# vbronetskyi/nclt-slam-project

Measured on AMD Instinct MI355X. Metric: relocalization frames/sec @640x480, 10k-landmark DB; Hamming-match HBM GB/s, higher is better.
Workload: dtype u8; 1 GPU; 640x480 BGR frames, 10000-record landmark DB (640000 descriptors, rows=fixed64), global relocalization tick per frame: ORB(500) + whole-DB mutual Hamming scan + top-25 PnP-RANSAC(200); frames resident in HBM, every frame's 96-byte result record written to pinned host memory by the tick's last kernel; distinct_frames=32, preroll_steps=20, streams=4, records=10000, descriptors=640000, parallelism=frames sharded across ranks, database replicated, no collective

## Files before the change

### nclt-slam-project_amd/csrc/reloc_ctx.hip

```cpp
#include <stdarg.h>
#include <stdlib.h>

#include "reloc_internal.h"

static thread_local char g_err[512] = "";

void reloc_set_error(const char *fmt, ...)
{
    va_list ap;
    va_start(ap, fmt);
    vsnprintf(g_err, sizeof(g_err), fmt, ap);
    va_end(ap);
}

RELOC_API const char *reloc_last_error(void) { return g_err; }

RELOC_API int reloc_device_count(void)
{
    int n = 0;
    if (hipGetDeviceCount(&n) != hipSuccess) return 0;
    return n;
}

template <typename T>
// ... 14 lines not shown
        pyr += ((w + 63) / 64 * 64) * h + 256;
    }
    c->pyr_bytes = pyr;
    rc |= dalloc(&c->pyr, pyr);
    rc |= dalloc(&c->blur, pyr);
    rc |= dalloc(&c->nms, pyr);
    rc |= dalloc(&c->rz_tab, (int64_t)NLEV * 2 * 2 * (c->max_w > c->max_h ? c->max_w : c->max_h));
    rc |= dalloc((char **)&c->pyr_tiles, (int64_t)((c->max_w + 15) / 16) * ((c->max_h + 15) / 16) * 128);
    rc |= dalloc(&c->hist, NLEV * 256);
    rc |= dalloc(&c->cand_cnt, NLEV);
    rc |= dalloc(&c->cand_key, (int64_t)NLEV * RELOC_ORB_STAGE1_CAP);
    rc |= dalloc(&c->cand_resp, (int64_t)NLEV * RELOC_ORB_STAGE1_CAP);
    rc |= dalloc(&c->kp_cnt, NLEV);
    rc |= dalloc(&c->kp_key, (int64_t)NLEV * RELOC_ORB_STAGE1_CAP);
    rc |= dalloc(&c->kp_resp, (int64_t)NLEV * RELOC_ORB_STAGE1_CAP);
    rc |= dalloc(&c->f_xy, mf * 2);
    rc |= dalloc(&c->f_size, mf);
    rc |= dalloc(&c->f_angle, mf);
    rc |= dalloc(&c->f_resp, mf);
    rc |= dalloc(&c->f_oct, mf);
    rc |= dalloc(&c->f_desc, mf * 32);
    rc |= dalloc(&c->f_count, 1);
    rc |= dalloc(&c->frame_img, (int64_t)c->max_w * c->max_h * 3);
    rc |= dalloc((char **)&c->orb_const, 1024);
    rc |= dalloc(&c->dbg_cut, NLEV);
    rc |= dalloc(&c->cand_ids, MAX_CAND);
    rc |= dalloc(&c->cand_n, 1);
    rc |= dalloc(&c->m_qidx, (int64_t)MAX_CAND * MAX_REC_ROWS);
    rc |= dalloc(&c->m_tidx, (int64_t)MAX_CAND * MAX_REC_ROWS);
    rc |= dalloc(&c->m_dist, (int64_t)MAX_CAND * MAX_REC_ROWS);
    rc |= dalloc(&c->m_n, MAX_CAND);
    rc |= dalloc(&c->p_obj, (int64_t)MAX_CAND * MAX_REC_ROWS * 3);
    rc |= dalloc(&c->p_img, (int64_t)MAX_CAND * MAX_REC_ROWS * 2);
    rc |= dalloc(&c->p_Rt, (int64_t)MAX_CAND * MAX_HYP * 12);
    rc |= dalloc(&c->p_cnt, (int64_t)MAX_CAND * MAX_HYP);
    rc |= dalloc(&c->p_inl, (int64_t)MAX_CAND * MAX_REC_ROWS);
    rc |= dalloc(&c->p_out, MAX_CAND);
    rc |= dalloc(&c->tick_res, 1);
    if (hipHostMalloc((void **)&c->tick_res_host, sizeof(TickResult), hipHostMallocDefault) != hipSuccess) {
        reloc_set_error("hipHostMalloc(result record) failed");
        c->tick_res_host = nullptr;
        rc |= RELOC_E_HIP;
    } else memset(c->tick_res_host, 0, sizeof(TickResult));
    rc |= dalloc(&c->accum_res, 1);
    rc |= dalloc(&c->tick_flags, 4);
    rc |= dalloc(&c->scan_ticket, (8 * 8 + 1) * 32);
    if (rc == 0 && hipMemset(c->scan_ticket, 0, (8 * 8 + 1) * 32 * 4) != hipSuccess) rc = RELOC_E_HIP;
    return rc;
}

int g_reloc_live_contexts = 0;

RELOC_API reloc_ctx *reloc_create(int device, int max_w, int max_h, int max_feat)
{
    int n = 0;
    if (hipGetDeviceCount(&n) != hipSuccess || n <= 0) {
        reloc_set_error("no HIP device available (libreloc_hip has no CPU fallback)");
        return nullptr;
    }
    if (device < 0 || device >= n || max_w < 64 || max_h < 64 || max_feat < 64) {
        reloc_set_error("reloc_create: bad arguments (device %d of %d, %dx%d, max_feat %d)", device, n,
                        max_w, max_h, max_feat);
        return nullptr;
    }
    if (hipSetDevice(device) != hipSuccess) {
        reloc_set_error("hipSetDevice(%d) failed", device);
        return nullptr;
    }
    reloc_ctx *c = new reloc_ctx();
    __atomic_add_fetch(&g_reloc_live_contexts, 1, __ATOMIC_RELAXED);
    c->device = device;
    c->max_w = max_w;
    c->max_h = max_h;
    c->max_feat = max_feat;
    hipDeviceProp_t prop;
    if (hipGetDeviceProperties(&prop, device) == hipSuccess) c->num_cu = prop.multiProcessorCount;
    if (hipStreamCreateWithFlags(&c->own_stream, hipStreamNonBlocking) != hipSuccess ||
        hipEventCreate(&c->t0) != hipSuccess || hipEventCreate(&c->t1) != hipSuccess) {
        reloc_set_error("stream/event creation failed");
        __atomic_sub_fetch(&g_reloc_live_contexts, 1, __ATOMIC_RELAXED);
        delete c;
        return nullptr;
    }
    c->stream = c->own_stream;
    c->prm.nfeatures = 500;
    c->prm.max_candidates = RELOC_MAX_CANDIDATES;
    c->prm.min_matches = RELOC_MIN_MATCHES;
    c->prm.min_inliers = RELOC_MIN_INLIERS;
    c->prm.ransac_iterations = RELOC_RANSAC_ITERATIONS;
    c->prm.global_max_candidates = RELOC_GLOBAL_MAX_CANDIDATES;
    c->prm.global_min_inliers = RELOC_GLOBAL_MIN_INLIERS;
    c->prm.accum_min_kpts = RELOC_ACCUM_MIN_KPTS;
    c->prm.candidate_radius_m = RELOC_CANDIDATE_RADIUS_M;
// ... 12 lines not shown
        if (const char *e = getenv("RELOC_SCAN_GENS")) c->scan_gens = atoi(e);
        if (const char *e = getenv("RELOC_LOCAL_TWO_STAGE")) c->local_two_stage = atoi(e) != 0;
    }
    if (ctx_alloc(c) != 0) {
        reloc_destroy(c);
        return nullptr;
    }
    return c;
}

RELOC_API void reloc_destroy(reloc_ctx *c)
{
    if (!c) return;
    (void)hipSetDevice(c->device);
    if (c->stream) (void)hipStreamSynchronize(c->stream);
    db_arrays_drop(c->db_share, c->db_desc, c->db_pts3d, c->db_kp2d, c->db_off, c->db_pose, c->db_xy_heading);
    void *ptrs[] = {c->pyr, c->blur, c->nms, c->rz_tab, c->pyr_tiles, c->hist, c->cand_cnt, c->cand_key, c->cand_resp,
                    c->kp_cnt, c->kp_key, c->kp_resp, c->f_xy, c->f_size, c->f_angle, c->f_resp, c->f_oct,
                    c->f_desc, c->f_count, c->frame_img, c->orb_const, c->dbg_cut, c->db_counts, c->topk_part, c->cand_ids, c->cand_n, c->m_qidx,
                    c->m_tidx, c->m_dist, c->m_n, c->p_obj, c->p_img, c->p_Rt, c->p_cnt, c->p_inl,
                    c->p_out, c->tick_res, c->accum_res, c->tick_flags, c->scan_ticket, c->clahe_plane, c->clahe_lut,
                    c->rect_xy };
    for (void *p : ptrs)
        if (p) (void)hipFree(p);
    if (c->tick_res_host) (void)hipHostFree(c->tick_res_host);
    {
        DbArena &a = c->db_slot[1 - c->db_sel];
        db_arrays_drop(a.share, a.desc, a.pts3d, a.kp2d, a.off, a.pose, a.xy_heading);
        if (a.counts) (void)hipFree(a.counts);
        if (a.topk_part) (void)hipFree(a.topk_part);
    }
    for (int i = 0; i < 8; ++i)
        if (c->scratch[i]) (void)hipFree(c->scratch[i]);
    for (int k = 0; k < RELOC_PROF_N; ++k)
        if (c->prof[k].init)
            for (int i = 0; i < RELOC_PROF_RING; ++i) {
                (void)hipEventDestroy(c->prof[k].a[i]);
                (void)hipEventDestroy(c->prof[k].b[i]);
            }
    if (c->t0) (void)hipEventDestroy(c->t0);
    if (c->t1) (void)hipEventDestroy(c->t1);
    if (c->own_stream) (void)hipStreamDestroy(c->own_stream);
    __atomic_sub_fetch(&g_reloc_live_contexts, 1, __ATOMIC_RELAXED);
    delete c;
}

RELOC_API int reloc_get_params(reloc_ctx *c, reloc_params *out)
{
    ARG_CHECK_CTX(c, out, "reloc_get_params");
    *out = c->prm;
    return RELOC_OK;
}

RELOC_API int reloc_set_params(reloc_ctx *c, const reloc_params *p)
{
    ARG_CHECK_CTX(c, p, "reloc_set_params");
// ... 2 lines not shown
    ARG_CHECK(p->global_max_candidates >= 1 && p->global_max_candidates <= MAX_CAND, "global_max_candidates must be in [1, 32]");
    ARG_CHECK(p->ransac_iterations >= 1 && p->ransac_iterations <= MAX_HYP, "ransac_iterations must be in [1, 1024]");
    ARG_CHECK(p->min_matches >= RELOC_PNP_SAMPLE && p->min_inliers >= 0 && p->global_min_inliers >= 0 && p->accum_min_kpts >= 1,
              "min_matches must be >= 4, inlier / keypoint gates non-negative");
    ARG_CHECK(p->candidate_radius_m >= 0 && p->heading_tol_deg >= 0 && p->heading_tol_deg <= 180 && p->ransac_reproj_px > 0 &&
                  p->ransac_confidence > 0 && p->ransac_confidence < 1 && p->consistency_m >= 0 && p->accum_min_dist_m >= 0,
              "a gate is out of range");
    ARG_CHECK((p->gray_coeff_bits == RELOC_GRAY_SHIFT || p->gray_coeff_bits == RELOC_GRAY15_SHIFT) && p->reserved0 == 0,
              "gray_coeff_bits must be 14 or 15, reserved0 must be 0");
    c->prm = *p;
    return RELOC_OK;
}

RELOC_API int reloc_set_stream(reloc_ctx *c, void *hip_stream)
{
    ARG_CHECK_CTX(c, true, "ctx is NULL");
    c->stream = hip_stream ? (hipStream_t)hip_stream : c->own_stream;
    return RELOC_OK;
}

RELOC_API int reloc_sync(reloc_ctx *c)
{
    ARG_CHECK_CTX(c, true, "ctx is NULL");
    HIP_TRY(hipStreamSynchronize(c->stream));
    return RELOC_OK;
}

RELOC_API void *reloc_dev_alloc(reloc_ctx *c, int64_t bytes)
{
    if (!c || bytes < 0) { reloc_set_error("reloc_dev_alloc: bad arguments"); return nullptr; }
    void *p = nullptr;
    (void)hipSetDevice(c->device);
    if (hipMalloc(&p, (size_t)(bytes > 0 ? bytes : 1)) != hipSuccess) {
        reloc_set_error("hipMalloc(%lld) failed", (long long)bytes);
        return nullptr;
    }
    return p;
}

RELOC_API int reloc_dev_free(reloc_ctx *c, void *p)
{
    ARG_CHECK_CTX(c, true, "ctx is NULL");
    if (p) HIP_TRY(hipFree(p));
    return RELOC_OK;
}

RELOC_API int reloc_h2d(reloc_ctx *c, void *dst, const void *src, int64_t bytes)
{
    ARG_CHECK_CTX(c, dst && src && bytes >= 0, "reloc_h2d");
    HIP_TRY(hipMemcpyAsync(dst, src, (size_t)bytes, hipMemcpyHostToDevice, c->stream));
    return RELOC_OK;
}

RELOC_API int reloc_d2d(reloc_ctx *c, void *dst, const void *src, int64_t bytes)
{
    ARG_CHECK_CTX(c, dst && src && bytes >= 0, "reloc_d2d");
    HIP_TRY(hipMemcpyAsync(dst, src, (size_t)bytes, hipMemcpyDeviceToDevice, c->stream));
    return RELOC_OK;
}

RELOC_API int reloc_set_exclusive(reloc_ctx *c, int on)
{
    ARG_CHECK_CTX(c, true, "ctx is NULL");
    c->exclusive_hint = on < 0 ? -1 : (on != 0);
// ... 8 lines not shown
        return nullptr;
    }
    return p;
}

RELOC_API int reloc_host_free(void *p)
{
    if (p) HIP_TRY(hipHostFree(p));
    return RELOC_OK;
}

RELOC_API void *reloc_get_stream(reloc_ctx *c) { return c ? (void *)c->stream : nullptr; }

RELOC_API int reloc_d2h(reloc_ctx *c, void *dst, const void *src, int64_t bytes)
{
    ARG_CHECK_CTX(c, dst && src && bytes >= 0, "reloc_d2h");
    HIP_TRY(hipMemcpyAsync(dst, src, (size_t)bytes, hipMemcpyDeviceToHost, c->stream));
    return RELOC_OK;
}

RELOC_API int reloc_timer_begin(reloc_ctx *c)
{
    ARG_CHECK_CTX(c, true, "ctx is NULL");
    HIP_TRY(hipEventRecord(c->t0, c->stream));
    return RELOC_OK;
}

RELOC_API int reloc_timer_end(reloc_ctx *c, float *ms)
{
    ARG_CHECK_CTX(c, ms, "reloc_timer_end");
    HIP_TRY(hipEventRecord(c->t1, c->stream));
// ... 76 lines not shown
```

### nclt-slam-project_amd/csrc/reloc_internal.h

```cpp
#pragma once
#include <hip/hip_runtime.h>
#include <stdint.h>
#include <stdio.h>
#include <string.h>

#include "../../include/reloc.h"
#include "../../include/reloc_spec.h"

#define RELOC_API extern "C" __attribute__((visibility("default")))
#define RELOC_PROF_RING 256

void reloc_set_error(const char *fmt, ...);

#define HIP_TRY(expr)                                                                      \
    do {                                                                                   \
        hipError_t e_ = (expr);                                                            \
        if (e_ != hipSuccess) {                                                            \
            reloc_set_error("%s failed: %s (%s:%d)", #expr, hipGetErrorString(e_), __FILE__, \
                            __LINE__);                                                     \
            return RELOC_E_HIP;                                                            \
        }                                                                                  \
    } while (0)

#define ARG_CHECK(cond, msg)                                 \
    do {                                                     \
        if (!(cond)) {                                       \
            reloc_set_error("bad argument: %s", msg);        \
            return RELOC_E_ARG;                              \
        }                                                    \
    } while (0)

#define ARG_CHECK_CTX(c, cond, msg)                           \
    do {                                                      \
        if (!(c) || !(cond)) {                                \
            reloc_set_error("bad argument: %s", msg);         \
            return RELOC_E_ARG;                               \
        }                                                     \
        (void)hipSetDevice((c)->device);                      \
    } while (0)

constexpr int NLEV = RELOC_ORB_NLEVELS;
constexpr int MAX_REC_ROWS = 4096;
constexpr int MAX_CAND = 32;
constexpr int MAX_HYP = 1024;
constexpr int64_t MAX_DB_RECORDS = 0xFFFFF;

#ifndef RELOC_SCAN_NUM_VGPR
#define RELOC_SCAN_NUM_VGPR 104
#endif
#if RELOC_SCAN_NUM_VGPR > 0
#define RELOC_SCAN_VGPR_ATTR __attribute__((amdgpu_num_vgpr(RELOC_SCAN_NUM_VGPR / 2)))
#else
#define RELOC_SCAN_VGPR_ATTR
#endif
#ifndef RELOC_SMALL_PRIO
#define RELOC_SMALL_PRIO 3
#endif
#define RELOC_SMALL_KERNEL_PRIO() __builtin_amdgcn_s_setprio(RELOC_SMALL_PRIO)

struct OrbLevel {
    int w, h;
    int stride;
    int64_t off;
    float scale;
    int quota;
};

struct TickResult {
// ... 235 lines not shown
    int32_t *cand_ids = nullptr;
    int32_t *cand_n = nullptr;
    int32_t *m_qidx = nullptr, *m_tidx = nullptr, *m_dist = nullptr, *m_n = nullptr;
    float *p_obj = nullptr, *p_img = nullptr;
    double *p_Rt = nullptr;
    int32_t *p_cnt = nullptr;
    int32_t *p_inl = nullptr;
    PnpOut *p_out = nullptr;
    int exclusive_hint = -1;
    bool local_two_stage = false;
    TickResult *tick_res = nullptr;
    TickResult *tick_res_host = nullptr;
    bool tick_failed = false;
    int32_t tick_seq = 0;
    TickResult *tick_res_ext = nullptr;
};

int reloc_scratch(reloc_ctx *ctx, int slot, int64_t bytes, void **out);
void reloc_prof_begin(reloc_ctx *ctx, int which);
void reloc_prof_end(reloc_ctx *ctx, int which);

void db_arrays_drop(DbShare *&share, uint8_t *&desc, float *&pts3d, float *&kp2d, int64_t *&off, double *&pose, double *&xyh);
extern int g_reloc_live_contexts;
static inline bool ctx_alone(const reloc_ctx *c)
{
    return c->exclusive_hint > 0 || (c->exclusive_hint < 0 && __atomic_load_n(&g_reloc_live_contexts, __ATOMIC_RELAXED) == 1);
}

constexpr int RELOC_BATCH_MAX = 8;

template <typename Fn>
// ... 18 lines not shown
```

### nclt-slam-project_amd/csrc/reloc_match.hip

```cpp
#include <stdlib.h>
#include <new>
#include <type_traits>
#include <utility>

#include "reloc_internal.h"

typedef uint32_t u32;

__device__ __forceinline__ u32 bcnt_acc(u32 x, u32 acc)
{
    u32 r;
    asm("v_bcnt_u32_b32 %0, %1, %2" : "=v"(r) : "v"(x), "v"(acc));
    return r;
}
__device__ __forceinline__ u32 min_u16(u32 a, u32 b)
{
    u32 r;
    asm("v_min_u16 %0, %1, %2" : "=v"(r) : "v"(a), "v"(b));
    return r;
}
template <u32 IDX>
__device__ __forceinline__ u32 key_fma(u32 d, u32 c128)
{
    u32 r;
// ... 448 lines not shown
        if (atomicAdd(&ticket_pool[words * TICKET_STRIDE], 1u) == gridDim.x - 1) {
            for (int x = 0; x <= words; ++x)
                __hip_atomic_store(&ticket_pool[x * TICKET_STRIDE], 0u, __ATOMIC_RELAXED, __HIP_MEMORY_SCOPE_AGENT);
        }
    }
}

template <int NJ, bool EMIT, int NW>
__global__ __launch_bounds__(64 * NW, 16 / NW) RELOC_SCAN_VGPR_ATTR void k_db_scan(
    const uint4 *__restrict__ db, const int64_t *__restrict__ off, const int32_t *__restrict__ rec_ids,
    const int32_t *__restrict__ n_ids_p, int n_ids_max, const uint4 *__restrict__ cur,
    const int32_t *__restrict__ n_cur_p, int n_cur_max, int max_rows, int32_t *__restrict__ counts,
    int32_t *__restrict__ m_qidx, int32_t *__restrict__ m_tidx, int32_t *__restrict__ m_dist,
    int32_t *__restrict__ m_n, int emit_stride, ScanMask mask, u32 *ticket, int quota, int n_bounded, int col_words)
{
    extern __shared__ u32 lds[];
    if constexpr (EMIT) RELOC_SMALL_KERNEL_PRIO();
    const int C = n_cur_p ? min(*n_cur_p, n_cur_max) : n_cur_max;
    if constexpr (EMIT)
        db_scan_body<NJ, true, NW>(lds, C, db, off, rec_ids, n_ids_p, n_ids_max, cur, max_rows, counts, m_qidx, m_tidx, m_dist, m_n,
                                   emit_stride, mask, ticket, quota);
    else
        db_count_body<NJ, NW>(lds, C, db, off, rec_ids, n_ids_p, n_ids_max, cur, max_rows, counts, mask, ticket, quota, n_bounded, col_words);
}

struct EmitFrame {
    const int32_t *rec_ids, *n_ids_p; const uint4 *cur; const int32_t *n_cur_p;
    int32_t *m_qidx, *m_tidx, *m_dist, *m_n; const float *g_xy; float *g_obj, *g_img;
};
struct EmitBatch { EmitFrame f[RELOC_BATCH_MAX]; };
static EmitFrame emit_frame(const reloc_ctx *c)
{
    EmitFrame F;
    F.rec_ids = c->cand_ids; F.n_ids_p = c->cand_n; F.cur = (const uint4 *)c->f_desc; F.n_cur_p = c->f_count;
    F.m_qidx = c->m_qidx; F.m_tidx = c->m_tidx; F.m_dist = c->m_dist; F.m_n = c->m_n; F.g_xy = c->f_xy; F.g_obj = c->p_obj; F.g_img = c->p_img;
    return F;
}

__global__ __launch_bounds__(256, 4) RELOC_SCAN_VGPR_ATTR void k_db_emit_batch(const uint4 *__restrict__ db, const int64_t *__restrict__ off, int n_ids_max,
                                                          int n_cur_max, int max_rows, int emit_stride, const float *__restrict__ g_pts3d,
                                                          EmitBatch bt)
{
    extern __shared__ u32 lds[];
    RELOC_SMALL_KERNEL_PRIO();
    const EmitFrame &F = bt.f[blockIdx.y];
    ScanMask mask;
    mask.g_pts3d = g_pts3d; mask.g_xy = F.g_xy; mask.g_obj = F.g_obj; mask.g_img = F.g_img;
    const int C = F.n_cur_p ? min(*F.n_cur_p, n_cur_max) : n_cur_max;
    db_scan_body<8, true, 4>(lds, C, db, off, F.rec_ids, F.n_ids_p, n_ids_max, F.cur, max_rows, nullptr, F.m_qidx, F.m_tidx, F.m_dist, F.m_n,
                             emit_stride, mask, nullptr, 0);
}

static int scan_lds_bytes(const char *who, int col_words, int max_rows, size_t &lds)
{
// ... 397 lines not shown
    if (n_ids_max <= 0) return RELOC_OK;
    if (n_cur_max > 65535) { reloc_set_error("db scan: more than 65535 current descriptors"); return RELOC_E_CAPACITY; }
    if (max_rows > MAX_REC_ROWS) { reloc_set_error("db scan: record larger than %d rows", MAX_REC_ROWS); return RELOC_E_CAPACITY; }
    if (max_rows < 1) max_rows = 1;
    const int nj = n > 1 || n_cur_max > 256 ? 8 : (n_cur_max <= 128 ? 2 : 4);
    const int cb = 64 * nj;
    const int ncb = (n_cur_max + cb - 1) / cb > 0 ? (n_cur_max + cb - 1) / cb : 1;
    size_t lds;
    if (int rc = scan_lds_bytes("db scan", ncb * cb, max_rows, lds)) return rc;
    const int grid = n_ids_max < c0->num_cu * 16 ? n_ids_max : c0->num_cu * 16;
    if (n == 1) {
        const EmitFrame &F = bt.f[0];
        ScanMask mask;
        mask.g_pts3d = g_pts3d; mask.g_xy = F.g_xy; mask.g_obj = F.g_obj; mask.g_img = F.g_img;
#define RELOC_LAUNCH_EMIT(NJ, NW)                                                                                            \
    hipLaunchKernelGGL((k_db_scan<NJ, true, NW>), dim3(grid), dim3(64 * NW), lds, c0->stream, (const uint4 *)db_desc, db_off, F.rec_ids, \
                       F.n_ids_p, n_ids_max, F.cur, F.n_cur_p, n_cur_max, max_rows, nullptr, F.m_qidx, F.m_tidx, F.m_dist, F.m_n,  \
                       emit_stride, mask, nullptr, 0, 0, ncb * cb)
        if (latency) {
            if (nj == 2) RELOC_LAUNCH_EMIT(2, 8); else if (nj == 4) RELOC_LAUNCH_EMIT(4, 8); else RELOC_LAUNCH_EMIT(8, 8);
        } else {
            if (nj == 2) RELOC_LAUNCH_EMIT(2, 4); else if (nj == 4) RELOC_LAUNCH_EMIT(4, 4); else RELOC_LAUNCH_EMIT(8, 4);
        }
#undef RELOC_LAUNCH_EMIT
    } else {
        hipLaunchKernelGGL(k_db_emit_batch, dim3(grid, n), dim3(256), lds, c0->stream, (const uint4 *)db_desc, db_off, n_ids_max,
                           n_cur_max, max_rows, emit_stride, g_pts3d, bt);
    }
    HIP_TRY(hipGetLastError());
    return RELOC_OK;
}

int launch_tick_emit(reloc_ctx *const *ctxs, int n, bool latency)
// ... 531 lines not shown
static void db_store_slot(reloc_ctx *ctx)
{
    DbArena &a = ctx->db_slot[ctx->db_sel];
    a.cap_records = ctx->db_cap_records; a.cap_rows = ctx->db_cap_rows; a.records = ctx->db_records; a.rows = ctx->db_rows;
    a.max_rows = ctx->db_max_rows; a.desc = ctx->db_desc; a.pts3d = ctx->db_pts3d; a.kp2d = ctx->db_kp2d; a.off = ctx->db_off;
    a.pose = ctx->db_pose; a.xy_heading = ctx->db_xy_heading; a.counts = ctx->db_counts; a.topk_part = ctx->topk_part;
    a.topk_blocks = ctx->topk_blocks;
    a.share = ctx->db_share;
}

RELOC_API int reloc_db_share(reloc_ctx *dst, reloc_ctx *src)
{
    ARG_CHECK_CTX(dst, src && src != dst, "reloc_db_share");
    if (src->device != dst->device) { reloc_set_error("reloc_db_share: contexts live on different devices"); return RELOC_E_ARG; }
    if (!db_ready(src)) { reloc_set_error("reloc_db_share: the source context has no database"); return RELOC_E_STATE; }
    HIP_TRY(hipStreamSynchronize(dst->stream));
    HIP_TRY(hipStreamSynchronize(src->stream));
    int32_t *counts = nullptr;
    unsigned long long *topk = nullptr;
    const int blocks = (int)((src->db_cap_records + 1023) / 1024);
    if (hipMalloc((void **)&counts, (size_t)src->db_cap_records * 4) != hipSuccess ||
        hipMalloc((void **)&topk, (size_t)blocks * 32 * sizeof(unsigned long long)) != hipSuccess) {
        if (counts) (void)hipFree(counts);
        reloc_set_error("reloc_db_share: scratch allocation failed");
        return RELOC_E_HIP;
    }
    if (dst->db_shared) db_unshare(dst);
    else {
        if (dst->db_counts) (void)hipFree(dst->db_counts);
        if (dst->topk_part) (void)hipFree(dst->topk_part);
// ... 100 lines not shown
```

### nclt-slam-project_amd/csrc/reloc_tick.hip

```cpp
#include <time.h>

#include "reloc_internal.h"

struct TickParams {
    double base_pose[7];
    double b2c_t[3];
    double b2c_R[9];
    int mode;
    int check_consistency;
    int n_records;
    int max_candidates, min_matches, min_inliers, global_min_inliers;
    double radius_m, cos_tol, reproj_max_px, global_reproj_max_px, consistency_m;
    int seq;
};

__device__ void rot_to_quat(const double R[9], double q[4])
{
    const double tr = R[0] + R[4] + R[8];
    double qx, qy, qz, qw;
    if (tr > 0) {
        const double s = 0.5 / sqrt(tr + 1.0);
        qw = 0.25 / s;
        qx = (R[7] - R[5]) * s; qy = (R[2] - R[6]) * s; qz = (R[3] - R[1]) * s;
    } else if (R[0] > R[4] && R[0] > R[8]) {
// ... 477 lines not shown
    p.check_consistency = check_consistency;
    p.n_records = (int)ctx->db_records;
    const reloc_params &q = ctx->prm;
    p.max_candidates = q.max_candidates; p.min_matches = q.min_matches; p.min_inliers = q.min_inliers;
    p.global_min_inliers = q.global_min_inliers;
    p.radius_m = q.candidate_radius_m; p.cos_tol = heading_cos_tol_host(ctx); p.reproj_max_px = q.reproj_max_px;
    p.global_reproj_max_px = q.global_reproj_max_px; p.consistency_m = q.consistency_m;
    p.seq = 0;
    return p;
}

static int tick_next_seq(reloc_ctx *ctx)
{
    ctx->tick_seq = ctx->tick_seq >= 0x7fffffff ? 1 : ctx->tick_seq + 1;
    ctx->tick_failed = false;
    return ctx->tick_seq;
}

struct SetCandBatch { int32_t *cand_ids[RELOC_BATCH_MAX], *cand_n[RELOC_BATCH_MAX], *flags[RELOC_BATCH_MAX]; };
__global__ void k_set_candidates_batch(const int32_t *__restrict__ ids, int k, SetCandBatch b, int flag)
{
    const int f = blockIdx.x;
    if (threadIdx.x == 0) {
        int m = 0;
        for (int i = 0; i < k; ++i)
            if (ids[f * k + i] >= 0) b.cand_ids[f][m++] = ids[f * k + i];
        *b.cand_n[f] = m;
        *b.flags[f] = flag;
    }
}
// ... 152 lines not shown
    int rc;
    if (cand_dev) {
        SetCandBatch sb;
        frame_slots(ctxs, n, [&](int f, reloc_ctx *c, int) { sb.cand_ids[f] = c->cand_ids; sb.cand_n[f] = c->cand_n; sb.flags[f] = c->tick_flags; });
        hipLaunchKernelGGL(k_set_candidates_batch, dim3(n), dim3(64), 0, c0->stream, cand_dev, k, sb, mode == RELOC_TICK_LOCAL ? 0 : 1);
    }
    if ((rc = launch_tick_emit(ctxs, n, latency))) return rc;
    if ((rc = pnp_run_candidates(ctxs, n, seeds, latency))) return rc;
    FinalBatch b;
    frame_slots(ctxs, n, [&](int f, reloc_ctx *c, int g) {
        b.f[f] = final_frame(c, base_poses + 7 * g, res_ext_base ? res_ext_base + g : c->tick_res_ext, f < n ? tick_next_seq(c) : 0);
    });
    return launch_tick_finalize(ctxs, n, b, make_tick_params(c0, base_poses, mode, check_consistency));
}

static int tick_run(reloc_ctx *const *ctxs, int n, const uint8_t *const *imgs, int w, int h, int order, const double *base_poses,
                    int mode, const uint64_t *seeds)
{
    reloc_ctx *c0 = ctxs[0];
    if (c0->max_feat > 65535) { reloc_set_error("tick: max_feat must be <= 65535"); return RELOC_E_CAPACITY; }
    const bool latency = tick_latency(ctxs, n, mode);
    int rc;
    if ((rc = orb_run(ctxs, n, imgs, w, h, w * 3, 3, order, c0->prm.nfeatures, latency))) return rc;
    if (mode != RELOC_TICK_GLOBAL)
        for (int f = 0; f < n; ++f) launch_candidates_local(ctxs[f], make_tick_params(ctxs[f], base_poses + 7 * f, mode, -1));
    if (mode != RELOC_TICK_LOCAL) {
        if ((rc = scan_counts(ctxs, n, base_poses, mode == RELOC_TICK_AUTO))) return rc;
        TopkBatch b;
        frame_slots(ctxs, n, [&](int f, reloc_ctx *c, int) { b.f[f] = topk_frame(c, c->cand_ids, nullptr, nullptr, mode == RELOC_TICK_AUTO); });
        launch_topk_counts(ctxs, n, b, c0->prm.global_max_candidates, 0);
    }
    return solve_run(ctxs, n, nullptr, 0, base_poses, mode, -1, seeds, nullptr);
}

static int scan_run(reloc_ctx *const *ctxs, int n, const uint8_t *const *imgs, int w, int h, int order, const double *base_poses,
                    const TopkBatch &out, int k, int id_base)
{
    int rc;
    if ((rc = orb_run(ctxs, n, imgs, w, h, w * 3, 3, order, ctxs[0]->prm.nfeatures, tick_latency(ctxs, n, RELOC_TICK_GLOBAL))))
        return rc;
    if ((rc = scan_counts(ctxs, n, base_poses, false))) return rc;
    launch_topk_counts(ctxs, n, out, k, id_base);
    HIP_TRY(hipGetLastError());
    return RELOC_OK;
}

RELOC_API int reloc_tick_dev(reloc_ctx *ctx, const uint8_t *img_dev, int w, int h, int order, const double base_pose[7],
                             int global_reloc, uint64_t seed)
{
    tick_mark_failed(&ctx, 1);
    ARG_CHECK_CTX(ctx, img_dev && base_pose && w >= 64 && h >= 64 && global_reloc >= 0 && global_reloc <= 2, "reloc_tick_dev");
    if (int rc = ctx_batch_check(&ctx, 1, "reloc_tick_dev")) return rc;
    return tick_run(&ctx, 1, &img_dev, w, h, order, base_pose, global_reloc, &seed);
}

RELOC_API int reloc_tick_batch_dev(reloc_ctx *const *ctxs, int n, const uint8_t *const *imgs_dev, int w, int h, int order,
                                   const double *base_poses, int global_reloc, const uint64_t *seeds)
{
    tick_mark_failed(ctxs, n);
    ARG_CHECK(ctxs && imgs_dev && base_poses && n >= 1 && n <= 8 && w >= 64 && h >= 64 && global_reloc >= 0 && global_reloc <= 2,
              "reloc_tick_batch_dev");
    for (int f = 0; f < n; ++f) ARG_CHECK(imgs_dev[f], "reloc_tick_batch_dev: NULL frame");
    if (int rc = ctx_batch_check(ctxs, n, "reloc_tick_batch_dev")) return rc;
    return tick_run(ctxs, n, imgs_dev, w, h, order, base_poses, global_reloc, seeds);
}

RELOC_API int reloc_tick_wait(reloc_ctx *ctx)
{
    ARG_CHECK_CTX(ctx, true, "ctx is NULL");
    if (ctx->tick_failed) {
        reloc_set_error("reloc_tick_wait: the last tick on this context failed before its result record was enqueued");
        return RELOC_E_STATE;
    }
    const int want = ctx->tick_seq;
    if (want == 0 || !ctx->tick_res_host) { HIP_TRY(hipStreamSynchronize(ctx->stream)); return RELOC_OK; }
    volatile int32_t *stamp = (volatile int32_t *)&ctx->tick_res_host->pad[0];
    struct timespec t0;
    clock_gettime(CLOCK_MONOTONIC, &t0);
    for (unsigned spin = 1;; ++spin) {
        if (*stamp == want) { __atomic_thread_fence(__ATOMIC_ACQUIRE); return RELOC_OK; }
        __builtin_ia32_pause();
        if ((spin & 0x3FF) == 0) {
            struct timespec t1;
            clock_gettime(CLOCK_MONOTONIC, &t1);
            if ((t1.tv_sec - t0.tv_sec) * 1000000000ll + (t1.tv_nsec - t0.tv_nsec) > 20000000ll) break;
        }
    }
    HIP_TRY(hipStreamSynchronize(ctx->stream));
    if (*stamp != want) { reloc_set_error("reloc_tick_wait: the stream drained without the tick's result record (a tick that failed to enqueue?)"); return RELOC_E_STATE; }
    return RELOC_OK;
}

RELOC_API int reloc_tick_result(reloc_ctx *ctx, double anchor_pose[7], int32_t *n_inl, float *reproj, int32_t *lm_idx,
                                int32_t *outcome, int32_t *n_candidates)
{
    ARG_CHECK_CTX(ctx, true, "ctx is NULL");
    { const int rc = reloc_tick_wait(ctx); if (rc) return rc; }
    const TickResult r = *ctx->tick_res_host;
    if (anchor_pose) for (int k = 0; k < 7; ++k) anchor_pose[k] = r.anchor_pose[k];
    if (n_inl) *n_inl = r.n_inl;
    if (reproj) *reproj = (float)r.reproj;
    if (lm_idx) *lm_idx = r.lm_idx;
    if (outcome) *outcome = r.outcome;
    if (n_candidates) *n_candidates = r.n_candidates;
    return RELOC_OK;
}

RELOC_API const void *reloc_tick_result_dev(reloc_ctx *ctx) { return ctx ? ctx->tick_res : nullptr; }

RELOC_API int reloc_tick_result_to(reloc_ctx *ctx, void *pinned_record)
{
    ARG_CHECK_CTX(ctx, true, "ctx is NULL");
    ctx->tick_res_ext = (TickResult *)pinned_record;
    return RELOC_OK;
}

RELOC_API int reloc_tick_result_ex(reloc_ctx *ctx, double anchor_pose[7], int32_t *n_inl, double *reproj, int32_t *lm_idx,
                                   int32_t *outcome, int32_t *n_candidates, int32_t *n_features, int32_t *relocating)
{
    ARG_CHECK_CTX(ctx, true, "ctx is NULL");
    { const int rc = reloc_tick_wait(ctx); if (rc) return rc; }
    const TickResult r = *ctx->tick_res_host;
    if (anchor_pose) for (int k = 0; k < 7; ++k) anchor_pose[k] = r.anchor_pose[k];
    if (n_inl) *n_inl = r.n_inl;
    if (reproj) *reproj = r.reproj;
    if (lm_idx) *lm_idx = r.lm_idx;
    if (outcome) *outcome = r.outcome;
    if (n_candidates) *n_candidates = r.n_candidates;
    if (n_features) *n_features = r.n_features;
    if (relocating) *relocating = r.relocating;
    return RELOC_OK;
}

RELOC_API int reloc_tick(reloc_ctx *ctx, const uint8_t *img, int w, int h, int order, const double base_pose[7],
                         int global_reloc, uint64_t seed, double anchor_pose[7], int32_t *n_inl, float *reproj,
                         int32_t *lm_idx, int32_t *outcome, int32_t *n_candidates)
{
    ARG_CHECK_CTX(ctx, img && base_pose && w >= 64 && h >= 64, "reloc_tick");
    if (w > ctx->max_w || h > ctx->max_h) { reloc_set_error("frame exceeds ctx capacity"); return RELOC_E_CAPACITY; }
    HIP_TRY(hipMemcpyAsync(ctx->frame_img, img, (size_t)w * h * 3, hipMemcpyHostToDevice, ctx->stream));
    int rc = reloc_tick_dev(ctx, ctx->frame_img, w, h, order, base_pose, global_reloc, seed);
    if (rc) return rc;
    return reloc_tick_result(ctx, anchor_pose, n_inl, reproj, lm_idx, outcome, n_candidates);
}

RELOC_API int reloc_tick_scan_dev(reloc_ctx *ctx, const uint8_t *img_dev, int w, int h, int order, const double base_pose[7],
                                  int32_t *topk_ids_dev, int32_t *topk_counts_dev, int k)
{
    ARG_CHECK_CTX(ctx, img_dev && topk_ids_dev && topk_counts_dev && k > 0 && k <= MAX_CAND && w >= 64 && h >= 64,
              "reloc_tick_scan_dev");
    if (int rc = ctx_batch_check(&ctx, 1, "reloc_tick_scan_dev")) return rc;
    TopkBatch out;
    frame_slots(&ctx, 1, [&](int f, reloc_ctx *c, int) { out.f[f] = topk_frame(c, topk_ids_dev, topk_counts_dev, nullptr, false); });
// ... 3 lines not shown
RELOC_API int reloc_tick_solve_dev(reloc_ctx *ctx, const int32_t *cand_ids_dev, int n_cand, const double base_pose[7],
                                   int check_consistency, uint64_t seed)
{
    tick_mark_failed(&ctx, 1);
    ARG_CHECK_CTX(ctx, cand_ids_dev && base_pose && n_cand >= 0 && n_cand <= MAX_CAND, "reloc_tick_solve_dev");
    if (int rc = ctx_batch_check(&ctx, 1, "reloc_tick_solve_dev")) return rc;
    return solve_run(&ctx, 1, cand_ids_dev, n_cand, base_pose, check_consistency ? RELOC_TICK_LOCAL : RELOC_TICK_GLOBAL,
                     check_consistency, &seed, nullptr);
}

RELOC_API int reloc_shard_scan_batch_dev(reloc_ctx *const *ctxs, int n, const uint8_t *const *imgs_dev, int w, int h, int order,
                                         const double *base_poses, int k, int64_t id_base, int32_t *scan_out_dev)
{
    int rc = ctx_batch_check(ctxs, n, "reloc_shard_scan_batch_dev");
    if (rc) return rc;
    ARG_CHECK(imgs_dev && scan_out_dev && k > 0 && k <= MAX_CAND && w >= 64 && h >= 64 && id_base >= 0 &&
              id_base + ctxs[0]->db_records <= 0x7fffffff, "reloc_shard_scan_batch_dev");
    for (int f = 0; f < n; ++f) ARG_CHECK(imgs_dev[f], "reloc_shard_scan_batch_dev: NULL frame");
    TopkBatch out;
    frame_slots(ctxs, n, [&](int f, reloc_ctx *c, int g) {
        int32_t *row = scan_out_dev + (size_t)g * (2 * k + 2);
        out.f[f] = topk_frame(c, row, row + k, row + 2 * k, false);
    });
    return scan_run(ctxs, n, imgs_dev, w, h, order, base_poses, out, k, (int)id_base);
}

__global__ __launch_bounds__(256) void k_shard_merge(const int32_t *__restrict__ all_scan, int world, int stride_w, int k, int id_base,
                                                     int n_local, int32_t *__restrict__ win_gid, int32_t *__restrict__ cand_local,
                                                     int32_t *__restrict__ n_feat)
{
// ... 32 lines not shown
    ARG_CHECK_CTX(ctx, all_scan_dev && win_gid_dev && cand_local_dev && n_feat_dev && world >= 1 && n >= 1 && n <= 8 && k > 0 &&
                  k <= MAX_CAND && stride_rank >= (int64_t)n * (2 * k + 2) && id_base >= 0 && n_local >= 0 &&
                  id_base + n_local <= 0x7fffffff && (int64_t)world * k <= 4096, "reloc_shard_merge_dev");
    hipLaunchKernelGGL(k_shard_merge, dim3(n), dim3(256), (size_t)world * k * sizeof(unsigned long long), ctx->stream, all_scan_dev, world,
                       (int)stride_rank, k, (int)id_base, (int)n_local, win_gid_dev, cand_local_dev, n_feat_dev);
    HIP_TRY(hipGetLastError());
    return RELOC_OK;
}

RELOC_API int reloc_shard_solve_batch_dev(reloc_ctx *const *ctxs, int n, const int32_t *cand_local_dev, int k,
                                          const double *base_poses, const uint64_t *seeds, void *res_out)
{
    tick_mark_failed(ctxs, n);
    int rc = ctx_batch_check(ctxs, n, "reloc_shard_solve_batch_dev");
    if (rc) return rc;
    ARG_CHECK(cand_local_dev && base_poses && res_out && k > 0 && k <= MAX_CAND, "reloc_shard_solve_batch_dev");
    return solve_run(ctxs, n, cand_local_dev, k, base_poses, RELOC_TICK_GLOBAL, 0, seeds, (TickResult *)res_out);
}

RELOC_API int reloc_tick_debug(reloc_ctx *ctx, int32_t *cand_ids, int32_t *n_cand, int32_t *n_matches, int32_t *n_inl,
                               int32_t *ok, double *reproj, double *Rt)
{
    ARG_CHECK_CTX(ctx, cand_ids && n_cand, "reloc_tick_debug");
    PnpOut po[MAX_CAND];
    HIP_TRY(hipMemcpyAsync(n_cand, ctx->cand_n, 4, hipMemcpyDeviceToHost, ctx->stream));
    HIP_TRY(hipMemcpyAsync(cand_ids, ctx->cand_ids, sizeof(int32_t) * MAX_CAND, hipMemcpyDeviceToHost, ctx->stream));
    HIP_TRY(hipMemcpyAsync(po, ctx->p_out, sizeof(po), hipMemcpyDeviceToHost, ctx->stream));
    HIP_TRY(hipStreamSynchronize(ctx->stream));
    for (int s = 0; s < *n_cand && s < MAX_CAND; ++s) {
        if (n_matches) n_matches[s] = po[s].n_matches;
// ... 8 lines not shown
```

Before: 7386 frames/s.

## Double-buffer per-tick feature buffers and overlap PnP solve with next frame's scan

```diff
diff --git a/nclt-slam-project_amd/csrc/reloc_ctx.hip b/nclt-slam-project_amd/csrc/reloc_ctx.hip
--- a/nclt-slam-project_amd/csrc/reloc_ctx.hip
+++ b/nclt-slam-project_amd/csrc/reloc_ctx.hip
@@ -52,18 +52,22 @@
     rc |= dalloc(&c->kp_cnt, NLEV);
     rc |= dalloc(&c->kp_key, (int64_t)NLEV * RELOC_ORB_STAGE1_CAP);
     rc |= dalloc(&c->kp_resp, (int64_t)NLEV * RELOC_ORB_STAGE1_CAP);
-    rc |= dalloc(&c->f_xy, mf * 2);
-    rc |= dalloc(&c->f_size, mf);
-    rc |= dalloc(&c->f_angle, mf);
-    rc |= dalloc(&c->f_resp, mf);
-    rc |= dalloc(&c->f_oct, mf);
-    rc |= dalloc(&c->f_desc, mf * 32);
-    rc |= dalloc(&c->f_count, 1);
+    for (reloc_ctx::TickSet &s : c->set) {
+        rc |= dalloc(&s.f_xy, mf * 2);
+        rc |= dalloc(&s.f_size, mf);
+        rc |= dalloc(&s.f_angle, mf);
+        rc |= dalloc(&s.f_resp, mf);
+        rc |= dalloc(&s.f_oct, mf);
+        rc |= dalloc(&s.f_desc, mf * 32);
+        rc |= dalloc(&s.f_count, 1);
+        rc |= dalloc(&s.cand_ids, MAX_CAND);
+        rc |= dalloc(&s.cand_n, 1);
+        rc |= dalloc(&s.tick_flags, 4);
+    }
+    ctx_select_set(c, 0);
     rc |= dalloc(&c->frame_img, (int64_t)c->max_w * c->max_h * 3);
     rc |= dalloc((char **)&c->orb_const, 1024);
     rc |= dalloc(&c->dbg_cut, NLEV);
-    rc |= dalloc(&c->cand_ids, MAX_CAND);
-    rc |= dalloc(&c->cand_n, 1);
     rc |= dalloc(&c->m_qidx, (int64_t)MAX_CAND * MAX_REC_ROWS);
     rc |= dalloc(&c->m_tidx, (int64_t)MAX_CAND * MAX_REC_ROWS);
     rc |= dalloc(&c->m_dist, (int64_t)MAX_CAND * MAX_REC_ROWS);
@@ -81,13 +85,37 @@
         rc |= RELOC_E_HIP;
     } else memset(c->tick_res_host, 0, sizeof(TickResult));
     rc |= dalloc(&c->accum_res, 1);
-    rc |= dalloc(&c->tick_flags, 4);
     rc |= dalloc(&c->scan_ticket, (8 * 8 + 1) * 32);
     if (rc == 0 && hipMemset(c->scan_ticket, 0, (8 * 8 + 1) * 32 * 4) != hipSuccess) rc = RELOC_E_HIP;
     return rc;
 }
 
 int g_reloc_live_contexts = 0;
+
+void ctx_select_set(reloc_ctx *c, int s)
+{
+    const reloc_ctx::TickSet &t = c->set[s];
+    c->cur = s;
+    c->f_xy = t.f_xy; c->f_size = t.f_size; c->f_angle = t.f_angle; c->f_resp = t.f_resp; c->f_oct = t.f_oct; c->f_desc = t.f_desc;
+    c->f_count = t.f_count; c->cand_ids = t.cand_ids; c->cand_n = t.cand_n; c->tick_flags = t.tick_flags;
+}
+
+int ctx_join(reloc_ctx *c)
+{
+    if (c->pending < 0) return RELOC_OK;
+    HIP_TRY(hipStreamWaitEvent(c->stream, c->solve_done[c->pending], 0));
+    c->pending = -1;
+    c->set_busy[0] = c->set_busy[1] = false;
+    return RELOC_OK;
+}
+
+int ctx_solve_stream(reloc_ctx *c, hipStream_t *out)
+{
+    if (c->stream != c->own_stream) { *out = c->own_stream; return RELOC_OK; }
+    if (!c->solve_own) HIP_TRY(hipStreamCreateWithFlags(&c->solve_own, hipStreamNonBlocking));
+    *out = c->solve_own;
+    return RELOC_OK;
+}
 
 RELOC_API reloc_ctx *reloc_create(int device, int max_w, int max_h, int max_feat)
 {
@@ -114,7 +142,11 @@
     hipDeviceProp_t prop;
     if (hipGetDeviceProperties(&prop, device) == hipSuccess) c->num_cu = prop.multiProcessorCount;
     if (hipStreamCreateWithFlags(&c->own_stream, hipStreamNonBlocking) != hipSuccess ||
-        hipEventCreate(&c->t0) != hipSuccess || hipEventCreate(&c->t1) != hipSuccess) {
+        hipEventCreate(&c->t0) != hipSuccess || hipEventCreate(&c->t1) != hipSuccess ||
+        hipEventCreateWithFlags(&c->scan_done[0], hipEventDisableTiming) != hipSuccess ||
+        hipEventCreateWithFlags(&c->scan_done[1], hipEventDisableTiming) != hipSuccess ||
+        hipEventCreateWithFlags(&c->solve_done[0], hipEventDisableTiming) != hipSuccess ||
+        hipEventCreateWithFlags(&c->solve_done[1], hipEventDisableTiming) != hipSuccess) {
         reloc_set_error("stream/event creation failed");
         __atomic_sub_fetch(&g_reloc_live_contexts, 1, __ATOMIC_RELAXED);
         delete c;
@@ -157,15 +189,21 @@
     if (!c) return;
     (void)hipSetDevice(c->device);
     if (c->stream) (void)hipStreamSynchronize(c->stream);
+    for (int s = 0; s < 2; ++s)
+        if (c->set_busy[s] && c->solve_done[s]) (void)hipEventSynchronize(c->solve_done[s]);
     db_arrays_drop(c->db_share, c->db_desc, c->db_pts3d, c->db_kp2d, c->db_off, c->db_pose, c->db_xy_heading);
     void *ptrs[] = {c->pyr, c->blur, c->nms, c->rz_tab, c->pyr_tiles, c->hist, c->cand_cnt, c->cand_key, c->cand_resp,
-                    c->kp_cnt, c->kp_key, c->kp_resp, c->f_xy, c->f_size, c->f_angle, c->f_resp, c->f_oct,
-                    c->f_desc, c->f_count, c->frame_img, c->orb_const, c->dbg_cut, c->db_counts, c->topk_part, c->cand_ids, c->cand_n, c->m_qidx,
+                    c->kp_cnt, c->kp_key, c->kp_resp, c->frame_img, c->orb_const, c->dbg_cut, c->db_counts, c->topk_part, c->m_qidx,
                     c->m_tidx, c->m_dist, c->m_n, c->p_obj, c->p_img, c->p_Rt, c->p_cnt, c->p_inl,
-                    c->p_out, c->tick_res, c->accum_res, c->tick_flags, c->scan_ticket, c->clahe_plane, c->clahe_lut,
+                    c->p_out, c->tick_res, c->accum_res, c->scan_ticket, c->clahe_plane, c->clahe_lut,
                     c->rect_xy };
     for (void *p : ptrs)
         if (p) (void)hipFree(p);
+    for (reloc_ctx::TickSet &s : c->set) {
+        void *sp[] = {s.f_xy, s.f_size, s.f_angle, s.f_resp, s.f_oct, s.f_desc, s.f_count, s.cand_ids, s.cand_n, s.tick_flags};
+        for (void *p : sp)
+            if (p) (void)hipFree(p);
+    }
     if (c->tick_res_host) (void)hipHostFree(c->tick_res_host);
     {
         DbArena &a = c->db_slot[1 - c->db_sel];
@@ -183,6 +221,11 @@
             }
     if (c->t0) (void)hipEventDestroy(c->t0);
     if (c->t1) (void)hipEventDestroy(c->t1);
+    for (int s = 0; s < 2; ++s) {
+        if (c->scan_done[s]) (void)hipEventDestroy(c->scan_done[s]);
+        if (c->solve_done[s]) (void)hipEventDestroy(c->solve_done[s]);
+    }
+    if (c->solve_own) (void)hipStreamDestroy(c->solve_own);
     if (c->own_stream) (void)hipStreamDestroy(c->own_stream);
     __atomic_sub_fetch(&g_reloc_live_contexts, 1, __ATOMIC_RELAXED);
     delete c;
@@ -215,15 +258,19 @@
 
 RELOC_API int reloc_set_stream(reloc_ctx *c, void *hip_stream)
 {
+    const int pend = c ? c->pending : -1;
     ARG_CHECK_CTX(c, true, "ctx is NULL");
     c->stream = hip_stream ? (hipStream_t)hip_stream : c->own_stream;
+    if (pend >= 0) HIP_TRY(hipStreamWaitEvent(c->stream, c->solve_done[pend], 0));
     return RELOC_OK;
 }
 
 RELOC_API int reloc_sync(reloc_ctx *c)
 {
+    const int pend = c ? c->pending : -1;
     ARG_CHECK_CTX(c, true, "ctx is NULL");
     HIP_TRY(hipStreamSynchronize(c->stream));
+    if (pend >= 0) HIP_TRY(hipEventSynchronize(c->solve_done[pend]));
     return RELOC_OK;
 }
 
@@ -248,7 +295,7 @@
 
 RELOC_API int reloc_h2d(reloc_ctx *c, void *dst, const void *src, int64_t bytes)
 {
-    ARG_CHECK_CTX(c, dst && src && bytes >= 0, "reloc_h2d");
+    ARG_CHECK_CTX_NOJOIN(c, dst && src && bytes >= 0, "reloc_h2d");
     HIP_TRY(hipMemcpyAsync(dst, src, (size_t)bytes, hipMemcpyHostToDevice, c->stream));
     return RELOC_OK;
 }
@@ -287,7 +334,9 @@
 
 RELOC_API int reloc_d2h(reloc_ctx *c, void *dst, const void *src, int64_t bytes)
 {
-    ARG_CHECK_CTX(c, dst && src && bytes >= 0, "reloc_d2h");
+    ARG_CHECK_CTX_NOJOIN(c, dst && src && bytes >= 0, "reloc_d2h");
+    if ((const char *)src >= (const char *)c->tick_res && (const char *)src < (const char *)(c->tick_res + 1))
+        if (int rc = ctx_join(c)) return rc;
     HIP_TRY(hipMemcpyAsync(dst, src, (size_t)bytes, hipMemcpyDeviceToHost, c->stream));
     return RELOC_OK;
 }
diff --git a/nclt-slam-project_amd/csrc/reloc_internal.h b/nclt-slam-project_amd/csrc/reloc_internal.h
--- a/nclt-slam-project_amd/csrc/reloc_internal.h
+++ b/nclt-slam-project_amd/csrc/reloc_internal.h
@@ -30,7 +30,7 @@
         }                                                    \
     } while (0)
 
-#define ARG_CHECK_CTX(c, cond, msg)                           \
+#define ARG_CHECK_CTX_NOJOIN(c, cond, msg)                    \
     do {                                                      \
         if (!(c) || !(cond)) {                                \
             reloc_set_error("bad argument: %s", msg);         \
@@ -38,6 +38,13 @@
         }                                                     \
         (void)hipSetDevice((c)->device);                      \
     } while (0)
+#define ARG_CHECK_CTX(c, cond, msg)                           \
+    do {                                                      \
+        ARG_CHECK_CTX_NOJOIN(c, cond, msg);                   \
+        if (int jrc_ = ctx_join(c)) return jrc_;              \
+    } while (0)
+struct reloc_ctx;
+int ctx_join(reloc_ctx *c);
 
 constexpr int NLEV = RELOC_ORB_NLEVELS;
 constexpr int MAX_REC_ROWS = 4096;
@@ -52,6 +59,14 @@
 #define RELOC_SCAN_VGPR_ATTR __attribute__((amdgpu_num_vgpr(RELOC_SCAN_NUM_VGPR / 2)))
 #else
 #define RELOC_SCAN_VGPR_ATTR
+#endif
+#ifndef RELOC_SCAN_EMIT_CAP
+#define RELOC_SCAN_EMIT_CAP 0
+#endif
+#if RELOC_SCAN_EMIT_CAP
+#define RELOC_EMIT_VGPR_ATTR RELOC_SCAN_VGPR_ATTR
+#else
+#define RELOC_EMIT_VGPR_ATTR
 #endif
 #ifndef RELOC_SMALL_PRIO
 #define RELOC_SMALL_PRIO 3
@@ -317,7 +332,30 @@
     bool tick_failed = false;
     int32_t tick_seq = 0;
     TickResult *tick_res_ext = nullptr;
-};
+
+    struct TickSet {
+        float *f_xy = nullptr, *f_size = nullptr, *f_angle = nullptr, *f_resp = nullptr;
+        int32_t *f_oct = nullptr;
+        uint8_t *f_desc = nullptr;
+        int32_t *f_count = nullptr, *cand_ids = nullptr, *cand_n = nullptr, *tick_flags = nullptr;
+    } set[2];
+    int cur = 0;
+    hipStream_t solve_own = nullptr;
+    hipEvent_t scan_done[2] = {}, solve_done[2] = {};
+    bool set_busy[2] = {false, false};
+    int pending = -1;
+    hipStream_t solve_last = nullptr;
+    bool tick_overlapped = false;
+};
+
+void ctx_select_set(reloc_ctx *c, int s);
+int ctx_solve_stream(reloc_ctx *c, hipStream_t *out);
+static inline int ctx_join_all(reloc_ctx *const *ctxs, int n)
+{
+    for (int f = 0; f < n; ++f)
+        if (int rc = ctx_join(ctxs[f])) return rc;
+    return RELOC_OK;
+}
 
 int reloc_scratch(reloc_ctx *ctx, int slot, int64_t bytes, void **out);
 void reloc_prof_begin(reloc_ctx *ctx, int which);
diff --git a/nclt-slam-project_amd/csrc/reloc_match.hip b/nclt-slam-project_amd/csrc/reloc_match.hip
--- a/nclt-slam-project_amd/csrc/reloc_match.hip
+++ b/nclt-slam-project_amd/csrc/reloc_match.hip
@@ -486,14 +486,25 @@
     int32_t *__restrict__ m_qidx, int32_t *__restrict__ m_tidx, int32_t *__restrict__ m_dist,
     int32_t *__restrict__ m_n, int emit_stride, ScanMask mask, u32 *ticket, int quota, int n_bounded, int col_words)
 {
+    static_assert(!EMIT, "the emit pass is k_db_scan_emit: it does not take the counting scans' register cap");
     extern __shared__ u32 lds[];
-    if constexpr (EMIT) RELOC_SMALL_KERNEL_PRIO();
     const int C = n_cur_p ? min(*n_cur_p, n_cur_max) : n_cur_max;
-    if constexpr (EMIT)
-        db_scan_body<NJ, true, NW>(lds, C, db, off, rec_ids, n_ids_p, n_ids_max, cur, max_rows, counts, m_qidx, m_tidx, m_dist, m_n,
-                                   emit_stride, mask, ticket, quota);
-    else
-        db_count_body<NJ, NW>(lds, C, db, off, rec_ids, n_ids_p, n_ids_max, cur, max_rows, counts, mask, ticket, quota, n_bounded, col_words);
+    db_count_body<NJ, NW>(lds, C, db, off, rec_ids, n_ids_p, n_ids_max, cur, max_rows, counts, mask, ticket, quota, n_bounded, col_words);
+}
+
+template <int NJ, int NW>
+__global__ __launch_bounds__(64 * NW, 16 / NW) RELOC_EMIT_VGPR_ATTR void k_db_scan_emit(
+    const uint4 *__restrict__ db, const int64_t *__restrict__ off, const int32_t *__restrict__ rec_ids,
+    const int32_t *__restrict__ n_ids_p, int n_ids_max, const uint4 *__restrict__ cur,
+    const int32_t *__restrict__ n_cur_p, int n_cur_max, int max_rows,
+    int32_t *__restrict__ m_qidx, int32_t *__restrict__ m_tidx, int32_t *__restrict__ m_dist,
+    int32_t *__restrict__ m_n, int emit_stride, ScanMask mask)
+{
+    extern __shared__ u32 lds[];
+    RELOC_SMALL_KERNEL_PRIO();
+    const int C = n_cur_p ? min(*n_cur_p, n_cur_max) : n_cur_max;
+    db_scan_body<NJ, true, NW>(lds, C, db, off, rec_ids, n_ids_p, n_ids_max, cur, max_rows, nullptr, m_qidx, m_tidx, m_dist, m_n,
+                               emit_stride, mask, nullptr, 0);
 }
 
 struct EmitFrame {
@@ -509,7 +520,7 @@
     return F;
 }
 
-__global__ __launch_bounds__(256, 4) RELOC_SCAN_VGPR_ATTR void k_db_emit_batch(const uint4 *__restrict__ db, const int64_t *__restrict__ off, int n_ids_max,
+__global__ __launch_bounds__(256, 4) RELOC_EMIT_VGPR_ATTR void k_db_emit_batch(const uint4 *__restrict__ db, const int64_t *__restrict__ off, int n_ids_max,
                                                           int n_cur_max, int max_rows, int emit_stride, const float *__restrict__ g_pts3d,
                                                           EmitBatch bt)
 {
@@ -937,9 +948,8 @@
         ScanMask mask;
         mask.g_pts3d = g_pts3d; mask.g_xy = F.g_xy; mask.g_obj = F.g_obj; mask.g_img = F.g_img;
 #define RELOC_LAUNCH_EMIT(NJ, NW)                                                                                            \
-    hipLaunchKernelGGL((k_db_scan<NJ, true, NW>), dim3(grid), dim3(64 * NW), lds, c0->stream, (const uint4 *)db_desc, db_off, F.rec_ids, \
-                       F.n_ids_p, n_ids_max, F.cur, F.n_cur_p, n_cur_max, max_rows, nullptr, F.m_qidx, F.m_tidx, F.m_dist, F.m_n,  \
-                       emit_stride, mask, nullptr, 0, 0, ncb * cb)
+    hipLaunchKernelGGL((k_db_scan_emit<NJ, NW>), dim3(grid), dim3(64 * NW), lds, c0->stream, (const uint4 *)db_desc, db_off, F.rec_ids, \
+                       F.n_ids_p, n_ids_max, F.cur, F.n_cur_p, n_cur_max, max_rows, F.m_qidx, F.m_tidx, F.m_dist, F.m_n, emit_stride, mask)
         if (latency) {
             if (nj == 2) RELOC_LAUNCH_EMIT(2, 8); else if (nj == 4) RELOC_LAUNCH_EMIT(4, 8); else RELOC_LAUNCH_EMIT(8, 8);
         } else {
@@ -1501,6 +1511,7 @@
     ARG_CHECK_CTX(dst, src && src != dst, "reloc_db_share");
     if (src->device != dst->device) { reloc_set_error("reloc_db_share: contexts live on different devices"); return RELOC_E_ARG; }
     if (!db_ready(src)) { reloc_set_error("reloc_db_share: the source context has no database"); return RELOC_E_STATE; }
+    if (int rc = ctx_join(src)) return rc;
     HIP_TRY(hipStreamSynchronize(dst->stream));
     HIP_TRY(hipStreamSynchronize(src->stream));
     int32_t *counts = nullptr;
diff --git a/nclt-slam-project_amd/csrc/reloc_tick.hip b/nclt-slam-project_amd/csrc/reloc_tick.hip
--- a/nclt-slam-project_amd/csrc/reloc_tick.hip
+++ b/nclt-slam-project_amd/csrc/reloc_tick.hip
@@ -515,6 +515,7 @@
 {
     ctx->tick_seq = ctx->tick_seq >= 0x7fffffff ? 1 : ctx->tick_seq + 1;
     ctx->tick_failed = false;
+    ctx->tick_overlapped = false;
     return ctx->tick_seq;
 }
 
@@ -697,14 +698,34 @@
     return launch_tick_finalize(ctxs, n, b, make_tick_params(c0, base_poses, mode, check_consistency));
 }
 
+static bool tick_overlaps(reloc_ctx *const *ctxs, int n, int mode) { return mode != RELOC_TICK_LOCAL && !tick_latency(ctxs, n, mode); }
+
 static int tick_run(reloc_ctx *const *ctxs, int n, const uint8_t *const *imgs, int w, int h, int order, const double *base_poses,
                     int mode, const uint64_t *seeds)
 {
     reloc_ctx *c0 = ctxs[0];
     if (c0->max_feat > 65535) { reloc_set_error("tick: max_feat must be <= 65535"); return RELOC_E_CAPACITY; }
-    const bool latency = tick_latency(ctxs, n, mode);
+    const bool latency = tick_latency(ctxs, n, mode), overlap = tick_overlaps(ctxs, n, mode);
+    hipStream_t main_q = c0->stream, solve_q = nullptr;
     int rc;
-    if ((rc = orb_run(ctxs, n, imgs, w, h, w * 3, 3, order, c0->prm.nfeatures, latency))) return rc;
+    if (!overlap) {
+        if ((rc = ctx_join_all(ctxs, n))) return rc;
+    } else {
+        if ((rc = ctx_solve_stream(c0, &solve_q))) return rc;
+        for (int f = 0; f < n; ++f) {
+            reloc_ctx *c = ctxs[f];
+            const int s = c->cur ^ 1;
+            if (c->set_busy[s]) {
+                HIP_TRY(hipStreamWaitEvent(main_q, c->solve_done[s], 0));
+                c->set_busy[s] = false;
+            }
+            ctx_select_set(c, s);
+        }
+    }
+    if ((rc = orb_run(ctxs, n, imgs, w, h, w * 3, 3, order, c0->prm.nfeatures, latency))) {
+        if (overlap) for (int f = 0; f < n; ++f) ctx_select_set(ctxs[f], ctxs[f]->cur ^ 1);
+        return rc;
+    }
     if (mode != RELOC_TICK_GLOBAL)
         for (int f = 0; f < n; ++f) launch_candidates_local(ctxs[f], make_tick_params(ctxs[f], base_poses + 7 * f, mode, -1));
     if (mode != RELOC_TICK_LOCAL) {
@@ -713,7 +734,28 @@
         frame_slots(ctxs, n, [&](int f, reloc_ctx *c, int) { b.f[f] = topk_frame(c, c->cand_ids, nullptr, nullptr, mode == RELOC_TICK_AUTO); });
         launch_topk_counts(ctxs, n, b, c0->prm.global_max_candidates, 0);
     }
-    return solve_run(ctxs, n, nullptr, 0, base_poses, mode, -1, seeds, nullptr);
+    if (!overlap) return solve_run(ctxs, n, nullptr, 0, base_poses, mode, -1, seeds, nullptr);
+    HIP_TRY(hipEventRecord(c0->scan_done[c0->cur], main_q));
+    HIP_TRY(hipStreamWaitEvent(solve_q, c0->scan_done[c0->cur], 0));
+    for (int f = 0; f < n; ++f) {
+        reloc_ctx *c = ctxs[f];
+        if (c->pending >= 0 && c->solve_last != solve_q) HIP_TRY(hipStreamWaitEvent(solve_q, c->solve_done[c->pending], 0));
+    }
+    c0->stream = solve_q;
+    rc = solve_run(ctxs, n, nullptr, 0, base_poses, mode, -1, seeds, nullptr);
+    c0->stream = main_q;
+    for (int f = 0; f < n; ++f) {
+        reloc_ctx *c = ctxs[f];
+        if (hipEventRecord(c->solve_done[c->cur], solve_q) != hipSuccess && !rc) {
+            reloc_set_error("hipEventRecord(solve_done) failed");
+            rc = RELOC_E_HIP;
+        }
+        c->set_busy[c->cur] = true;
+        c->pending = c->cur;
+        c->solve_last = solve_q;
+        if (!rc) c->tick_overlapped = true;
+    }
+    return rc;
 }
 
 static int scan_run(reloc_ctx *const *ctxs, int n, const uint8_t *const *imgs, int w, int h, int order, const double *base_poses,
@@ -732,7 +774,7 @@
                              int global_reloc, uint64_t seed)
 {
     tick_mark_failed(&ctx, 1);
-    ARG_CHECK_CTX(ctx, img_dev && base_pose && w >= 64 && h >= 64 && global_reloc >= 0 && global_reloc <= 2, "reloc_tick_dev");
+    ARG_CHECK_CTX_NOJOIN(ctx, img_dev && base_pose && w >= 64 && h >= 64 && global_reloc >= 0 && global_reloc <= 2, "reloc_tick_dev");
     if (int rc = ctx_batch_check(&ctx, 1, "reloc_tick_dev")) return rc;
     return tick_run(&ctx, 1, &img_dev, w, h, order, base_pose, global_reloc, &seed);
 }
@@ -750,7 +792,7 @@
 
 RELOC_API int reloc_tick_wait(reloc_ctx *ctx)
 {
-    ARG_CHECK_CTX(ctx, true, "ctx is NULL");
+    ARG_CHECK_CTX_NOJOIN(ctx, true, "ctx is NULL");
     if (ctx->tick_failed) {
         reloc_set_error("reloc_tick_wait: the last tick on this context failed before its result record was enqueued");
         return RELOC_E_STATE;
@@ -769,7 +811,8 @@
             if ((t1.tv_sec - t0.tv_sec) * 1000000000ll + (t1.tv_nsec - t0.tv_nsec) > 20000000ll) break;
         }
     }
-    HIP_TRY(hipStreamSynchronize(ctx->stream));
+    if (ctx->tick_overlapped && ctx->pending >= 0) HIP_TRY(hipEventSynchronize(ctx->solve_done[ctx->pending]));
+    else HIP_TRY(hipStreamSynchronize(ctx->stream));
     if (*stamp != want) { reloc_set_error("reloc_tick_wait: the stream drained without the tick's result record (a tick that failed to enqueue?)"); return RELOC_E_STATE; }
     return RELOC_OK;
 }
@@ -777,7 +820,7 @@
 RELOC_API int reloc_tick_result(reloc_ctx *ctx, double anchor_pose[7], int32_t *n_inl, float *reproj, int32_t *lm_idx,
                                 int32_t *outcome, int32_t *n_candidates)
 {
-    ARG_CHECK_CTX(ctx, true, "ctx is NULL");
+    ARG_CHECK_CTX_NOJOIN(ctx, true, "ctx is NULL");
     { const int rc = reloc_tick_wait(ctx); if (rc) return rc; }
     const TickResult r = *ctx->tick_res_host;
     if (anchor_pose) for (int k = 0; k < 7; ++k) anchor_pose[k] = r.anchor_pose[k];
@@ -793,7 +836,7 @@
 
 RELOC_API int reloc_tick_result_to(reloc_ctx *ctx, void *pinned_record)
 {
-    ARG_CHECK_CTX(ctx, true, "ctx is NULL");
+    ARG_CHECK_CTX_NOJOIN(ctx, true, "ctx is NULL");
     ctx->tick_res_ext = (TickResult *)pinned_record;
     return RELOC_OK;
 }
@@ -801,7 +844,7 @@
 RELOC_API int reloc_tick_result_ex(reloc_ctx *ctx, double anchor_pose[7], int32_t *n_inl, double *reproj, int32_t *lm_idx,
                                    int32_t *outcome, int32_t *n_candidates, int32_t *n_features, int32_t *relocating)
 {
-    ARG_CHECK_CTX(ctx, true, "ctx is NULL");
+    ARG_CHECK_CTX_NOJOIN(ctx, true, "ctx is NULL");
     { const int rc = reloc_tick_wait(ctx); if (rc) return rc; }
     const TickResult r = *ctx->tick_res_host;
     if (anchor_pose) for (int k = 0; k < 7; ++k) anchor_pose[k] = r.anchor_pose[k];
@@ -819,7 +862,7 @@
                          int global_reloc, uint64_t seed, double anchor_pose[7], int32_t *n_inl, float *reproj,
                          int32_t *lm_idx, int32_t *outcome, int32_t *n_candidates)
 {
-    ARG_CHECK_CTX(ctx, img && base_pose && w >= 64 && h >= 64, "reloc_tick");
+    ARG_CHECK_CTX_NOJOIN(ctx, img && base_pose && w >= 64 && h >= 64, "reloc_tick");
     if (w > ctx->max_w || h > ctx->max_h) { reloc_set_error("frame exceeds ctx capacity"); return RELOC_E_CAPACITY; }
     HIP_TRY(hipMemcpyAsync(ctx->frame_img, img, (size_t)w * h * 3, hipMemcpyHostToDevice, ctx->stream));
     int rc = reloc_tick_dev(ctx, ctx->frame_img, w, h, order, base_pose, global_reloc, seed);
@@ -853,6 +896,7 @@
 {
     int rc = ctx_batch_check(ctxs, n, "reloc_shard_scan_batch_dev");
     if (rc) return rc;
+    if ((rc = ctx_join_all(ctxs, n))) return rc;
     ARG_CHECK(imgs_dev && scan_out_dev && k > 0 && k <= MAX_CAND && w >= 64 && h >= 64 && id_base >= 0 &&
               id_base + ctxs[0]->db_records <= 0x7fffffff, "reloc_shard_scan_batch_dev");
     for (int f = 0; f < n; ++f) ARG_CHECK(imgs_dev[f], "reloc_shard_scan_batch_dev: NULL frame");
@@ -915,6 +959,7 @@
     tick_mark_failed(ctxs, n);
     int rc = ctx_batch_check(ctxs, n, "reloc_shard_solve_batch_dev");
     if (rc) return rc;
+    if ((rc = ctx_join_all(ctxs, n))) return rc;
     ARG_CHECK(cand_local_dev && base_poses && res_out && k > 0 && k <= MAX_CAND, "reloc_shard_solve_batch_dev");
     return solve_run(ctxs, n, cand_local_dev, k, base_poses, RELOC_TICK_GLOBAL, 0, seeds, (TickResult *)res_out);
 }
```

New measurement: 5977 frames/s. 19.1% lower.
